# Ichoran/dbce-video-cpp

Measured on AMD Instinct MI355X. Metric: frames/s + raw-pixel GB/s, 4096x3072 U8 encode+decode round-trip, higher is better.
Workload: dtype u8

## Files before the change

### dbde-video-cpp_amd/csrc/dbde_kernels.hip

```cpp
#include "dbde_kernels.h"

#include "dbde_bits.h"
#include "dbde_device.h"


namespace dbde {

#ifndef DBDE_DIAG_LATE
#define DBDE_DIAG_LATE 34
#endif
#ifdef DBDE_DIAG
#define SF_DECL uint64_t sfd[10] = {0, 0, 0, 0, 0, 0, 0, 0, 0, 0}
#define SF_MARK(i) do { if (threadIdx.x == 0) sfd[i] = wall_clock64(); } while (0)
#define SF_DRAIN() asm volatile("s_waitcnt vmcnt(0) lgkmcnt(0)" ::: "memory")
#define SF_FLUSH(diag, last)                                                                          \
    do {                                                                                              \
        if (threadIdx.x == 0 && (diag)) {                                                             \
            atomicMax(&(diag)[0], ~(unsigned long long)sfd[0]);                                       \
            for (int i_ = 1; i_ < 10; i_++) atomicAdd(&(diag)[i_], (unsigned long long)sfd[i_]);      \
            atomicAdd(&(diag)[10], 1ull);                                                             \
            atomicMax(&(diag)[11], (unsigned long long)sfd[last]);                                    \
            atomicMax(&(diag)[12], (unsigned long long)sfd[0]);                                       \
            atomicAdd(&(diag)[13], (unsigned long long)sfd[0]);                                       \
        }                                                                                             \
// ... 1869 lines not shown
        uint32_t dsum = 0, dbad = 0;
        if (2u * (uint32_t)tid < n_tiles) { const uint32_t d = darr[te]; dsum += d; dbad |= d > 8u ? 1u : 0u; }
        if (2u * (uint32_t)tid + 1u < n_tiles) { const uint32_t d = darr[te + 1u]; dsum += d; dbad |= d > 8u ? 1u : 0u; }
        dsum = wave_sum(dsum);
        const bool wbad = __any((int)dbad);
        if (lane == 0) { s_idx[wave][0] = dsum; s_idx[wave][1] = wbad ? 1u : 0u; }
        __syncthreads();
        SF_MARK(1);
        unsigned long long *rec = p.fuse_rec + (size_t)f * cpf;
        const unsigned long long tag = (unsigned long long)p.fuse_epoch << 32;
        if (tid == 0 && !((p.fuse_flags & 1u) && (cf & 1u))) {
            uint32_t mine = 0, mbad = 0;
#pragma unroll
            for (int k = 0; k < G::kWaves; k++) { mine += s_idx[k][0]; mbad |= s_idx[k][1]; }
            __hip_atomic_store(&rec[cf], tag | ((unsigned long long)mbad << 31) | mine, __ATOMIC_RELAXED, __HIP_MEMORY_SCOPE_AGENT);
        }
        {
            const uint64_t t_start = wall_clock64();
            uint32_t before = 0, total = 0, flag = 0;
            auto take = [&](const uint32_t base, unsigned long long w) __attribute__((always_inline)) {
                const uint32_t k = base + (uint32_t)lane;
                bool got = k >= cpf || (w >> 32) == (tag >> 32);
                for (;;) {
                    if (__all((int)got)) break;
                    if (wall_clock64() - t_start > 3000ull) {
                        uint64_t miss = __ballot((int)!got);
                        while (miss) {
                            const uint32_t kk = (uint32_t)__builtin_ctzll(miss);
                            miss &= miss - 1ull;
                            const uint32_t c_lo = dec_chunk_begin(p.geom, base + kk), c_hi = dec_chunk_begin(p.geom, base + kk + 1u);
                            uint32_t sm = 0, bd = 0;
#pragma unroll
                            for (uint32_t j = 0; j < 8u; j += 4u) {
                                const uint32_t q = c_lo + (uint32_t)lane * 8u + j;
                                if (q < c_hi) {
                                    uint32_t x;
                                    __builtin_memcpy(&x, darr + q, 4);
                                    const uint32_t keep = c_hi - q;
                                    if (keep < 4u) x &= 0xFFFFFFFFu >> (8u * (4u - keep));
                                    bd |= depth_bytes_bad(x, 1u);
                                    sm += __builtin_amdgcn_sad_u8(x, 0u, 0u);
                                }
                            }
                            sm = wave_sum(sm);
                            const bool anyb = __any((int)(bd != 0u));
                            if ((uint32_t)lane == kk) { w = tag | ((unsigned long long)(anyb ? 1u : 0u) << 31) | sm; got = true; }
                        }
                        break;
                    }
                    __builtin_amdgcn_s_sleep(1);
                    if (!got) { w = __hip_atomic_load(&rec[k], __ATOMIC_RELAXED, __HIP_MEMORY_SCOPE_AGENT); got = (w >> 32) == (tag >> 32); }
                }
                const uint32_t v = k < cpf ? (uint32_t)w & 0x7FFFFFFFu : 0u;
                total += v;
                before += k < cf ? v : 0u;
                flag |= k < cpf ? (uint32_t)(w >> 31) & 1u : 0u;
            };
            constexpr uint32_t kStride = 64u * (uint32_t)G::kWaves;
            for (uint32_t base = 64u * (uint32_t)wave; base < cpf; base += 2u * kStride) {
                const uint32_t kA = base + (uint32_t)lane, kB = kA + kStride;
                const unsigned long long wA = kA < cpf ? __hip_atomic_load(&rec[kA], __ATOMIC_RELAXED, __HIP_MEMORY_SCOPE_AGENT) : 0ull;
                const unsigned long long wB = kB < cpf ? __hip_atomic_load(&rec[kB], __ATOMIC_RELAXED, __HIP_MEMORY_SCOPE_AGENT) : 0ull;
                take(base, wA);
                if (base + kStride < cpf) take(base + kStride, wB);
            }
            before = wave_sum(before); total = wave_sum(total);
            const bool anyflag = __any((int)flag);
            if (lane == 0) { s_idx[wave][2] = before; s_idx[wave][3] = total | (anyflag ? 0x80000000u : 0u); }
        }
        SF_MARK(2);
        __syncthreads();
        uint32_t before = 0, total = 0, flag = 0;
#pragma unroll
        for (int k = 0; k < G::kWaves; k++) { before += s_idx[k][2]; total += s_idx[k][3] & 0x7FFFFFFFu; flag |= s_idx[k][3] >> 31; }
        uint32_t mine = 0;
#pragma unroll
        for (int k = 0; k < G::kWaves; k++) mine += s_idx[k][0];
        const bool okf = nb == (int32_t)T && nm == (int32_t)T && n64 == (int32_t)total && !flag &&
                         in_extent(foff, need + 8ull * total, p.stream_bytes);
        if (record) {
            res->u64s = (field == 2u && okf) ? 2u : 0xFFFFFFFFu;
            res->pad_ = 0; res->index = index; res->elapsed_ns = elapsed;
            res->consumed = okf ? need + 8ull * total : 20ull;
        }
        if (!okf) return;
        w_begin = before;
        w_end = before + mine;
        __syncthreads();
        SF_MARK(3);
    } else {
        const uint32_t ok = p.frame_ok[f];
        const uint32_t *co = p.chunk_off + (size_t)f * (p.chunks_per_frame + 1u) + cf;
        w_begin = co[0]; w_end = co[1];
        asm volatile("" :: "s"(ok), "s"(w_begin), "s"(w_end), "s"((uint32_t)foff));
        if (!ok) return;
    }

    const uint32_t t0 = t_begin + 2u * (uint32_t)tid;
    const bool hasA = 2u * (uint32_t)tid < n_tiles, hasB = 2u * (uint32_t)tid + 1u < n_tiles;
    const uint8_t *depth_arr = fb + 24;
    const uint8_t *min_arr = fb + 28 + p.T;

    const uint32_t chunk_words = w_end - w_begin;
    const uint8_t *src = fb + 32ull + 2ull * p.T + 8ull * w_begin;
    const uint32_t shift = (uint32_t)(reinterpret_cast<uintptr_t>(src) & 15u);
    const uint8_t *asrc = src - shift;
    const uint32_t n16 = (shift + 8u * chunk_words + 15u) >> 4;
    const bool swz = chunk_words == 8u * n_tiles || chunk_words == 4u * n_tiles || chunk_words == 7u * n_tiles;
    const uint32_t n16r = (n16 + 15u) & ~15u;
    const uint8_t *s_end = p.stream + p.stream_bytes;
    const uint32_t n16_dma = (asrc + 16ull * n16 <= s_end) ? n16 : n16 - 1u;
#pragma unroll
    for (int j = 0; j < G::kPieces; j++) {
        const uint32_t i = (uint32_t)tid + (uint32_t)j * G::kThreads;
        const uint32_t src_slot = swz ? swz16(i) : i;
        if (i < n16r && src_slot < n16_dma) {
            const uint32_t wave_slot0 = (uint32_t)j * G::kThreads + (uint32_t)wave * 64u;
            __builtin_amdgcn_global_load_lds(
                (const __attribute__((address_space(1))) void *)(asrc + 16ull * src_slot),
                (__attribute__((address_space(3))) void *)(&s_in[2u * wave_slot0]), 16, 0, 2 );
        }
    }
    if (n16_dma != n16 && tid < 16) {
        const uint8_t *b = asrc + 16ull * n16_dma + (uint32_t)tid;
        reinterpret_cast<uint8_t *>(s_in)[16u * (swz ? swz16(n16_dma) : n16_dma) + (uint32_t)tid] = b < s_end ? *b : (uint8_t)0;
    }
    SF_MARK(4);
    uint32_t dA = 0, dB = 0, mA = 0, mB = 0;
    if (hasB && ((reinterpret_cast<uintptr_t>(depth_arr + t0) | reinterpret_cast<uintptr_t>(min_arr + t0)) & 1u) == 0u) {
        const uint32_t d2 = *reinterpret_cast<const uint16_t *>(depth_arr + t0);
        const uint32_t m2 = *reinterpret_cast<const uint16_t *>(min_arr + t0);
        dA = d2 & 0xFFu; dB = d2 >> 8; mA = m2 & 0xFFu; mB = m2 >> 8;
    } else {
        if (hasA) { dA = depth_arr[t0]; mA = min_arr[t0]; }
        if (hasB) { dB = depth_arr[t0 + 1]; mB = min_arr[t0 + 1]; }
    }

    asm volatile("s_waitcnt vmcnt(0) lgkmcnt(0)" ::: "memory");
    SF_MARK(5);
    uint32_t chunk_total;
    const uint32_t incl = block_scan_incl<G::kWaves>(dA + dB, s_wave_tot, lane, wave, chunk_total);
    SF_MARK(6);
    const uint32_t offA = incl - (dA + dB), offB = offA + dA;

    uint32_t va[16], vb[16];
    const uint8_t *s_img = reinterpret_cast<const uint8_t *>(s_in);
    const uint32_t bA = shift + 8u * offA, bB = shift + 8u * offB;
    const bool all8 = swz && (shift & 7u) == 0u && __all((int)((dA == 8u || !hasA) && (dB == 8u || !hasB)));
    const bool flat = __all((int)((dA | dB) == 0u));
    if (flat) {
#pragma unroll
        for (int i = 0; i < 16; i++) { va[i] = mA * 0x01010101u; vb[i] = mB * 0x01010101u; }
    } else if (all8) {
        unpack_tile_d8_from_lds(s_img, bA, mA, va);
        unpack_tile_d8_from_lds(s_img, bB, mB, vb);
    } else {
        if (swz) {
            unpack_tile_from_lds<true>(s_img, bA, dA, mA, va);
            unpack_tile_from_lds<true>(s_img, bB, dB, mB, vb);
        } else {
            unpack_tile_from_lds<false>(s_img, bA, dA, mA, va);
            unpack_tile_from_lds<false>(s_img, bB, dB, mB, vb);
        }
    }

    SF_MARK(7);
    uint8_t *img = p.images + (size_t)f * p.frame_pixels;
    if (IMG == kImgDirect) {
        if (hasA) {
            const uint32_t ty = t0 / p.w, tx = t0 - ty * p.w;
            uint8_t *base = img + (size_t)(8u * tx);
#pragma unroll
            for (int r = 0; r < 8; r++) {
                const int yy = 8 * (int)ty + r;
                if (yy < p.H) {
                    u32x4_t o;
                    o[0] = va[2 * r]; o[1] = va[2 * r + 1]; o[2] = vb[2 * r]; o[3] = vb[2 * r + 1];
                    __builtin_nontemporal_store(o, reinterpret_cast<u32x4_t *>(base + (size_t)yy * (size_t)p.W));
                }
            }
        }
        SF_MARK(8);
        SF_DRAIN();
        SF_MARK(9);
        if (INDEX == kIdxFused) SF_FLUSH(p.diag, 9);
        return;
    }

    if (IMG == kImgTiles) {
        if (hasA) store_tile_generic(img, p.W, p.H, p.w, t0, va);
        if (hasB) store_tile_generic(img, p.W, p.H, p.w, t0 + 1u, vb);
        return;
    }

    const bool whole_rows = p.geom.pieces == 1u;
    const uint32_t ty0 = whole_rows ? t_begin / p.w : cf / p.geom.pieces;
    const uint32_t tx0 = whole_rows ? 0u : (cf - ty0 * p.geom.pieces) * kChunkTiles;
    const uint32_t wspan = whole_rows ? p.w : n_tiles;
    const uint32_t Wu = (uint32_t)p.W, y0 = 8u * ty0;
    const uint32_t tile_rows = whole_rows ? n_tiles / p.w : 1u;
    const uint32_t y_end = y0 + 8u * tile_rows < (uint32_t)p.H ? y0 + 8u * tile_rows : (uint32_t)p.H;
    const uint32_t x_valid = Wu - 8u * tx0 < 8u * wspan ? Wu - 8u * tx0 : 8u * wspan;
    uint8_t *g_first = img + (size_t)y0 * (size_t)p.W + (size_t)(8u * tx0);
    const uint32_t g7 = (uint32_t)(reinterpret_cast<uintptr_t>(g_first) & 127u);
    uint8_t *s_px = reinterpret_cast<uint8_t *>(s_in);
    const bool a8 = ((g7 | Wu) & 7u) == 0u;
    if (!a8 && !whole_rows) {
        if (hasA) store_tile_generic(img, p.W, p.H, p.w, t0, va);
        if (hasB) store_tile_generic(img, p.W, p.H, p.w, t0 + 1u, vb);
        return;
    }
    if (whole_rows && ((uint32_t)(reinterpret_cast<uintptr_t>(img) & 15u) | (Wu & 15u)) == 0u && chunk_words != 8u * n_tiles) {
        if (hasA) {
            const uint32_t iD = 2u * (uint32_t)tid, rowD = iD / wspan, colD = iD - rowD * wspan;
            uint8_t *base = img + (size_t)(8u * colD);
#pragma unroll
            for (int r = 0; r < 8; r++) {
                const uint32_t yy = y0 + 8u * rowD + (uint32_t)r;
                if (yy < (uint32_t)p.H) {
                    u32x4_t o;
                    o[0] = va[2 * r]; o[1] = va[2 * r + 1]; o[2] = vb[2 * r]; o[3] = vb[2 * r + 1];
                    __builtin_nontemporal_store(o, reinterpret_cast<u32x4_t *>(base + (size_t)yy * (size_t)p.W));
                }
            }
        }
        return;
    }
    __syncthreads();
    const uint32_t iA = 2u * (uint32_t)tid;
    const uint32_t rowA = iA / wspan, colA = iA - rowA * wspan;
    const uint32_t rowB = colA + 1u == wspan ? rowA + 1u : rowA, colB = colA + 1u == wspan ? 0u : colA + 1u;
    const uint32_t nA = 8u * colA + 8u <= x_valid ? 8u : x_valid - 8u * colA;
    const uint32_t nB = 8u * colB + 8u <= x_valid ? 8u : x_valid - 8u * colB;
    const bool all_rows = y0 + 8u * tile_rows <= (uint32_t)p.H;
    const bool plain = all_rows && __all((int)((!hasA || nA == 8u) && (!hasB || nB == 8u)));
    if (a8) {
        const uint32_t l_pitch = 8u * kChunkTiles + 128u;
        const uint32_t aA = whole_rows ? g7 + 8u * rowA * Wu + 8u * colA : 8u * colA;
        const uint32_t aB = whole_rows ? g7 + 8u * rowB * Wu + 8u * colB : 8u * colB;
        auto row_term = [&](uint32_t r) -> uint32_t {
            return whole_rows ? r * Wu : ((g7 + r * Wu) & 127u) + r * l_pitch;
        };
        if (plain) {
            if (hasA) {
#pragma unroll
                for (int r = 0; r < 8; r++) lds_store_u64_any(s_px, aA + row_term((uint32_t)r), va[2 * r], va[2 * r + 1]);
            }
            if (hasB) {
#pragma unroll
                for (int r = 0; r < 8; r++) lds_store_u64_any(s_px, aB + row_term((uint32_t)r), vb[2 * r], vb[2 * r + 1]);
            }
        } else {
#pragma unroll
            for (int r = 0; r < 8; r++) {
                const uint32_t rt = row_term((uint32_t)r);
                if (hasA && y0 + 8u * rowA + (uint32_t)r < y_end) {
                    if (nA == 8u) lds_store_u64_any(s_px, aA + rt, va[2 * r], va[2 * r + 1]);
                    else lds_store_bytes(s_px, aA + rt, ((uint64_t)va[2 * r + 1] << 32) | va[2 * r], nA);
                }
                if (hasB && y0 + 8u * rowB + (uint32_t)r < y_end) {
                    if (nB == 8u) lds_store_u64_any(s_px, aB + rt, vb[2 * r], vb[2 * r + 1]);
                    else lds_store_bytes(s_px, aB + rt, ((uint64_t)vb[2 * r + 1] << 32) | vb[2 * r], nB);
                }
            }
        }
        asm volatile("s_waitcnt lgkmcnt(0)" ::: "memory");
        __syncthreads();
        const uint32_t n_ranges = whole_rows ? 1u : y_end - y0;
        for (uint32_t s = 0; s < n_ranges; s++) {
            uint8_t *g0 = g_first + (size_t)s * Wu;
            const uint32_t bytes = whole_rows ? (y_end - y0) * Wu : x_valid;
            const uint32_t head = (uint32_t)(reinterpret_cast<uintptr_t>(g0) & 127u);
            uint8_t *a0 = g0 - head;
            const uint8_t *l0 = s_px + (whole_rows ? 0u : s * l_pitch);
            const uint32_t n_blocks = (head + bytes + 15u) >> 4;
            for (uint32_t j = (uint32_t)tid; j < n_blocks; j += (uint32_t)G::kThreads) {
                if (16u * j + 16u <= head || 16u * j >= head + bytes) continue;
                if (16u * j >= head && 16u * j + 16u <= head + bytes) {
                    const u32x4_t q = *reinterpret_cast<const u32x4_t *>(l0 + 16u * j);
                    __builtin_nontemporal_store(q, reinterpret_cast<u32x4_t *>(a0 + 16ull * j));
                } else {
#pragma unroll
                    for (uint32_t b = 0; b < 16u; b++) {
                        const uint32_t o = 16u * j + b;
                        if (o >= head && o < head + bytes) a0[o] = l0[o];
                    }
                }
            }
        }
        return;
    }
    const uint32_t P = 8u * wspan + 16u;
    const uint32_t aA = 8u * rowA * P + 8u * colA, aB = 8u * rowB * P + 8u * colB;
    if (hasA) {
#pragma unroll
        for (int r = 0; r < 8; r++) lds_store_u64_any(s_px, aA + (uint32_t)r * P, va[2 * r], va[2 * r + 1]);
    }
    if (hasB) {
#pragma unroll
        for (int r = 0; r < 8; r++) lds_store_u64_any(s_px, aB + (uint32_t)r * P, vb[2 * r], vb[2 * r + 1]);
    }
    asm volatile("s_waitcnt lgkmcnt(0)" ::: "memory");
    __syncthreads();
    if (hasA && colA <= 1u) {
#pragma unroll
        for (int r = 0; r < 8; r++) {
            const uint32_t ry = 8u * rowA + (uint32_t)r;
            if (ry != 0u) lds_store_u64_any(s_px, (ry - 1u) * P + Wu + 8u * colA, va[2 * r], va[2 * r + 1]);
        }
    }
    if (hasB && colB <= 1u) {
#pragma unroll
        for (int r = 0; r < 8; r++) {
            const uint32_t ry = 8u * rowB + (uint32_t)r;
            if (ry != 0u) lds_store_u64_any(s_px, (ry - 1u) * P + Wu + 8u * colB, vb[2 * r], vb[2 * r + 1]);
        }
    }
    asm volatile("s_waitcnt lgkmcnt(0)" ::: "memory");
    __syncthreads();
    {
        const uint32_t bytes = (y_end - y0) * Wu;
        uint8_t *a0 = g_first - g7;
        const uint32_t n_blocks = (g7 + bytes + 15u) >> 4;
        const uint32_t lds0 = (uint32_t)(uintptr_t)(__attribute__((address_space(3))) const uint8_t *)s_px;
        const uint32_t last_n = (g7 + bytes) & 15u;
        for (uint32_t j0 = (uint32_t)tid; j0 < n_blocks; j0 += 4u * (uint32_t)G::kThreads) {
            uint64_t d01[4], d23[4];
            uint32_t d4[4], a[4];
            bool live[4];
#pragma unroll
            for (uint32_t k = 0; k < 4u; k++) {
                const uint32_t j = j0 + k * (uint32_t)G::kThreads;
                live[k] = j < n_blocks && 16u * j + 16u > g7;
                const uint32_t o = live[k] && 16u * j > g7 ? 16u * j - g7 : 0u;
                uint32_t col;
                const uint32_t row = div_magic(o, Wu, p.magic_W, col);
                a[k] = lds0 + row * P + col;
                const uint32_t a4 = a[k] & ~3u;
                asm volatile("ds_read2_b32 %0, %3 offset1:1\n\tds_read2_b32 %1, %3 offset0:2 offset1:3\n\tds_read_b32 %2, %3 offset:16"
                             : "=&v"(d01[k]), "=&v"(d23[k]), "=&v"(d4[k]) : "v"(a4) : "memory");
            }
            asm volatile("s_waitcnt lgkmcnt(0)" : "+v"(d01[0]), "+v"(d23[0]), "+v"(d4[0]), "+v"(d01[1]), "+v"(d23[1]), "+v"(d4[1]),
                         "+v"(d01[2]), "+v"(d23[2]), "+v"(d4[2]), "+v"(d01[3]), "+v"(d23[3]), "+v"(d4[3]) :: "memory");
#pragma unroll
            for (uint32_t k = 0; k < 4u; k++) {
                const uint32_t j = j0 + k * (uint32_t)G::kThreads;
                const uint32_t w0 = (uint32_t)d01[k], w1 = (uint32_t)(d01[k] >> 32), w2 = (uint32_t)d23[k], w3 = (uint32_t)(d23[k] >> 32);
                u32x4_t q;
                q[0] = __builtin_amdgcn_alignbyte(w1, w0, a[k]);
                q[1] = __builtin_amdgcn_alignbyte(w2, w1, a[k]);
                q[2] = __builtin_amdgcn_alignbyte(w3, w2, a[k]);
                q[3] = __builtin_amdgcn_alignbyte(d4[k], w3, a[k]);
                if (!live[k]) continue;
                const bool first = 16u * j < g7, last = 16u * j + 16u > g7 + bytes;
                if (!first && !last) {
                    __builtin_nontemporal_store(q, reinterpret_cast<u32x4_t *>(a0 + 16ull * j));
                } else {
                    uint8_t *dst = first ? g_first : a0 + 16ull * j;
                    uint32_t n = first ? 16u - (g7 & 15u) : last_n;
                    if (first && last) n = bytes;
                    uint64_t lo = ((uint64_t)q[1] << 32) | q[0], hi = ((uint64_t)q[3] << 32) | q[2];
                    if (n & 8u) { store_u64_any(dst, lo); dst += 8; lo = hi; }
                    if (n & 4u) { const uint32_t v = (uint32_t)lo; __builtin_memcpy(dst, &v, 4); dst += 4; lo >>= 32; }
                    if (n & 2u) { const uint16_t v = (uint16_t)lo; __builtin_memcpy(dst, &v, 2); dst += 2; lo >>= 16; }
                    if (n & 1u) *dst = (uint8_t)lo;
                }
            }
        }
    }
}

struct MidMeta {
    uint32_t d, mn;
    uint32_t nb, nm, n64;
};

#ifndef DBDE_MID_WAVES
#define DBDE_MID_WAVES 6
#endif
template <int THREADS, bool STAGED>
__global__ __launch_bounds__(THREADS, THREADS == 1024 ? 4 : DBDE_MID_WAVES) void decode_mid_kernel(DecParams p) {
    constexpr int NW = THREADS / 64;
    __shared__ uint32_t s_tot[2][NW];
    __shared__ uint32_t s_incl[2][THREADS];
    constexpr uint32_t kMidSlot = 80u;
    __shared__ __attribute__((aligned(16))) uint8_t s_lds[THREADS * kMidSlot];
    __shared__ uint32_t s_ok[THREADS];
    __shared__ uint32_t s_bad[2];
    const uint32_t tid = threadIdx.x, lane = tid & 63u, wave = tid >> 6;
    const uint32_t T = p.T, fpw = (uint32_t)THREADS / T;
    const uint32_t fl = tid / T, t = tid - fl * T;
    const uint32_t n_frames = p.n_chunks;
    const uint32_t n_groups = (n_frames + fpw - 1u) / fpw, G = gridDim.x;
    const bool slot = fl < fpw;
    const uint32_t first = slot ? fl * T : 0u;
    const uint64_t need = 32ull + 2ull * T;
    const uint8_t *s_end = p.stream + p.stream_bytes;
    const uint32_t ty = t / p.w, tx = t - ty * p.w;
    const uint32_t Wu = (uint32_t)p.W, x0 = 8u * tx;
    const uint32_t rm = Wu - x0 < 8u ? Wu - x0 : 8u;
    const uint32_t rv = (uint32_t)p.H - 8u * ty < 8u ? (uint32_t)p.H - 8u * ty : 8u;
    const uint32_t tile_off = 8u * ty * Wu + x0;
    const bool want_results = p.results != nullptr;

    auto is_active = [&](uint32_t g) -> bool { return slot && g < n_groups && g * fpw + fl < n_frames; };
    auto get_foff = [&](uint32_t g) -> uint64_t { return is_active(g) ? p.frame_offsets[g * fpw + fl] : 0ull; };
    auto get_meta = [&](uint32_t g, uint64_t foff) -> MidMeta {
        MidMeta m;
        m.d = 0; m.mn = 0; m.nb = 0; m.nm = 0; m.n64 = 0;
        const bool active = is_active(g);
        const uint8_t *fb = p.stream + foff;
        if (active && in_extent(foff, need, p.stream_bytes)) {
            m.d = fb[24u + t]; m.mn = fb[28u + T + t];
            __builtin_memcpy(&m.nb, fb + 20, 4); __builtin_memcpy(&m.nm, fb + 24 + T, 4); __builtin_memcpy(&m.n64, fb + 28 + 2ull * T, 4);
        }
        return m;
    };

    if (STAGED && tid == 0u) { s_bad[0] = 0u; s_bad[1] = 0u; }
    uint32_t g = blockIdx.x;
    uint64_t foff_cur = get_foff(g), foff_nxt = get_foff(g + G);
    auto settle = [&](const MidMeta &x, uint32_t &dm, uint32_t &n64x) {
        dm = x.d | (x.mn << 8);
        n64x = ((int32_t)x.nb == (int32_t)T && (int32_t)x.nm == (int32_t)T) ? x.n64 : 0xFFFFFFFFu;
    };
    uint32_t dm, n64x;
    settle(get_meta(g, foff_cur), dm, n64x);
    for (uint32_t par = 0; g < n_groups; g += G, par ^= 1u) {
        MidMeta m_nxt = get_meta(g + G, foff_nxt);
        uint64_t foff_nn = get_foff(g + 2u * G);
        const bool active = is_active(g);
        const uint32_t f = g * fpw + fl;
        const uint64_t foff = foff_cur;
        const bool in_range = active && in_extent(foff, need, p.stream_bytes);
        const uint32_t d = dm & 0xFFu, mn = dm >> 8;
        const uint32_t item = in_range ? (d | (d > 8u ? 1u << 20 : 0u)) : 0u;
        const uint32_t w_incl = wave_scan_incl(item);
        s_incl[par][tid] = w_incl;
        if (lane == 63u) s_tot[par][wave] = w_incl;
        lds_barrier();
        if (STAGED && tid == 0u) s_bad[par ^ 1u] = 0u;
        auto pref = [&](uint32_t x) -> uint32_t {
            uint32_t a = s_incl[par][x];
#pragma unroll
            for (int k = 0; k < NW - 1; k++) a += (uint32_t)k < (x >> 6) ? s_tot[par][k] : 0u;
            return a;
        };
        const uint32_t base = first ? pref(active ? first - 1u : 0u) : 0u;
        const uint32_t upto = pref(active ? first + T - 1u : 0u);
        const uint32_t mine = pref(tid);
        const uint32_t total = (upto - base) & 0xFFFFFu, n_bad = (upto - base) >> 20;
        const uint32_t prefix = (mine - item - base) & 0xFFFFFu;
        const bool ok = in_range && n64x == total && n_bad == 0u && in_extent(foff, need + 8ull * total, p.stream_bytes);
        uint32_t h_field = 0;
        uint64_t h_index = 0, h_elapsed = 0;
        const bool record = active && t == 0u && want_results;
        if (record && in_extent(foff, 20, p.stream_bytes)) {
            const uint8_t *fb = p.stream + foff;
            __builtin_memcpy(&h_field, fb, 4); __builtin_memcpy(&h_index, fb + 4, 8); __builtin_memcpy(&h_elapsed, fb + 12, 8);
        }
        const uint8_t *pay = p.stream + foff + need + 8ull * prefix;
        const uint32_t poff = (uint32_t)(reinterpret_cast<uintptr_t>(pay) & 3u);
        const uint8_t *psrc = pay - poff;
        const uint32_t npc_all = (8u * d + poff + 15u) >> 4;
        const bool whole = ok && d != 0u && psrc + 16u * npc_all <= s_end;
        const uint32_t npc = whole ? npc_all : 0u;
        u32x4_t q0 = {0u, 0u, 0u, 0u}, q1 = q0, q2 = q0, q3 = q0, q4 = q0;
        if (npc > 0u) __builtin_memcpy(&q0, psrc, 16);
        if (npc > 1u) __builtin_memcpy(&q1, psrc + 16, 16);
        if (npc > 2u) __builtin_memcpy(&q2, psrc + 32, 16);
        if (npc > 3u) __builtin_memcpy(&q3, psrc + 48, 16);
        if (npc > 4u) __builtin_memcpy(&q4, psrc + 64, 16);
        asm volatile("" : "+v"(q0), "+v"(q1), "+v"(q2), "+v"(q3), "+v"(q4),
                          "+v"(m_nxt.d), "+v"(m_nxt.mn), "+v"(m_nxt.nb), "+v"(m_nxt.nm), "+v"(m_nxt.n64), "+v"(foff_nn),
                          "+v"(h_field), "+v"(h_index), "+v"(h_elapsed) :: "memory");
        const uint32_t slot = kMidSlot * tid;
        {
            u32x4_t *sl = reinterpret_cast<u32x4_t *>(s_lds + slot);
            if (npc > 0u) sl[0] = q0;
            if (npc > 1u) sl[1] = q1;
            if (npc > 2u) sl[2] = q2;
            if (npc > 3u) sl[3] = q3;
            if (npc > 4u) sl[4] = q4;
        }
        if (ok && d != 0u && !whole) {
            for (uint32_t b = 0; b < 8u * d; b++) s_lds[slot + poff + b] = pay[b];
        }
        uint32_t v[16];
#pragma unroll
        for (int i = 0; i < 16; i++) v[i] = 0;
        if (ok) unpack_tile_from_lds<false>(s_lds, slot + poff, d, mn, v);
        if (STAGED) lds_barrier();
        if (ok) {
            uint8_t *dst = p.images + (size_t)f * p.frame_pixels + tile_off;
            const uint32_t px0 = ((uint32_t)(reinterpret_cast<uintptr_t>(p.images) + (size_t)(g * fpw) * p.frame_pixels) & 15u) +
                                 fl * (uint32_t)p.frame_pixels + tile_off;
#pragma unroll
            for (int r = 0; r < 8; r++) {
                const uint32_t lo = v[2 * r], hi = v[2 * r + 1];
                if (STAGED) {
                    if ((uint32_t)r < rv) {
                        const uint32_t a = px0 + (uint32_t)r * Wu;
                        if ((Wu & 7u) == 0u) lds_store_u64_any(s_lds, a, lo, hi);
                        else {
                            *reinterpret_cast<uint32_t *>(s_lds + a) = lo;
                            if (rm == 8u) *reinterpret_cast<uint32_t *>(s_lds + a + 4u) = hi;
                        }
                    }
                } else if ((uint32_t)r < rv) {
                    uint8_t *row = dst + (size_t)r * Wu;
                    const uint64_t q = ((uint64_t)hi << 32) | lo;
                    if (rm == 8u) store_u64_any(row, q);
                    else {
#pragma unroll
                        for (uint32_t k = 0; k < 8u; k++)
                            if (k < rm) row[k] = (uint8_t)(q >> (8u * k));
                    }
                }
            }
        }
        if (STAGED) {
            if (active && t == 0u) { s_ok[fl] = ok ? 1u : 0u; if (!ok) s_bad[par] = 1u; }
            lds_barrier();
            const uint32_t P = (uint32_t)p.frame_pixels;
            const uint32_t nfr = n_frames - g * fpw < fpw ? n_frames - g * fpw : fpw;
            uint8_t *g0 = p.images + (size_t)(g * fpw) * p.frame_pixels;
            const uint32_t sh = (uint32_t)(reinterpret_cast<uintptr_t>(g0) & 15u);
            const uint32_t nbytes = nfr * P;
            if (s_bad[par] == 0u) {
                const uint32_t n_blocks = (sh + nbytes + 15u) >> 4;
                for (uint32_t j = tid; j < n_blocks; j += (uint32_t)THREADS) {
                    uint8_t *dst = g0 - sh + 16ull * j;
                    if (16u * j >= sh && 16u * j + 16u <= sh + nbytes) {
                        const u32x4_t q = *reinterpret_cast<const u32x4_t *>(s_lds + 16u * j);
                        __builtin_nontemporal_store(q, reinterpret_cast<u32x4_t *>(dst));
                    } else {
#pragma unroll
                        for (uint32_t k = 0; k < 4u; k++) {
                            const uint32_t o = 16u * j + 4u * k;
                            if (o >= sh && o < sh + nbytes) *reinterpret_cast<uint32_t *>(dst + 4u * k) = *reinterpret_cast<const uint32_t *>(s_lds + o);
                        }
                    }
                }
            } else {
                for (uint32_t u = tid; 4u * u < nbytes; u += (uint32_t)THREADS) {
                    const uint32_t o = 4u * u;
                    if (s_ok[o / P]) *reinterpret_cast<uint32_t *>(g0 + o) = *reinterpret_cast<const uint32_t *>(s_lds + sh + o);
                }
            }
        }
        if (record) {
            FrameResultDev *r = reinterpret_cast<FrameResultDev *>(p.results) + f;
            r->u64s = (h_field == 2u && ok) ? 2u : 0xFFFFFFFFu;
            r->pad_ = 0;
            r->index = h_index;
            r->elapsed_ns = f64_to_u64_x86(__longlong_as_double((long long)h_elapsed));
            r->consumed = ok ? need + 8ull * total : 20ull;
        }
        foff_cur = foff_nxt; foff_nxt = foff_nn;
        settle(m_nxt, dm, n64x);
    }
}

void decode_mid_blocks_per_cu(int (&per_cu)[2][3]) {
    auto ask = [](auto kernel, int threads) {
        int n = 0;
        if (hipOccupancyMaxActiveBlocksPerMultiprocessor(&n, kernel, threads, 0) != hipSuccess || n < 1) n = 1;
        return n;
    };
    per_cu[0][0] = ask(decode_mid_kernel<256, false>, 256);
    per_cu[0][1] = ask(decode_mid_kernel<512, false>, 512);
    per_cu[0][2] = ask(decode_mid_kernel<1024, false>, 1024);
    per_cu[1][0] = ask(decode_mid_kernel<256, true>, 256);
    per_cu[1][1] = ask(decode_mid_kernel<512, true>, 512);
    per_cu[1][2] = ask(decode_mid_kernel<1024, true>, 1024);
}

hipError_t launch_decode_mid(const DecParams &p, uint32_t n_frames, uint32_t n_cu, const int (&per_cu)[2][3], hipStream_t s) {
    DecParams q = p;
    q.n_chunks = n_frames;
    const uint32_t th = mid_decode_threads_for(p.T), per_wg = th / p.T;
    uint32_t groups = (n_frames + per_wg - 1u) / per_wg;
    const bool staged = p.W % 4 == 0 && (reinterpret_cast<uintptr_t>(p.images) & 3u) == 0u;
    auto go = [&](auto kernel, uint32_t threads) {
        const int wg = per_cu[staged ? 1 : 0][threads == 256u ? 0 : (threads == 512u ? 1 : 2)];
        const uint32_t resident = n_cu ? n_cu * (uint32_t)wg : 3u;
        hipLaunchKernelGGL(kernel, dim3(groups < resident ? groups : resident), dim3(threads), 0, s, q);
    };
    if (staged) {
        if (th == 256u) go(decode_mid_kernel<256, true>, 256u);
        else if (th == 512u) go(decode_mid_kernel<512, true>, 512u);
        else go(decode_mid_kernel<1024, true>, 1024u);
    } else {
        if (th == 256u) go(decode_mid_kernel<256, false>, 256u);
        else if (th == 512u) go(decode_mid_kernel<512, false>, 512u);
        else go(decode_mid_kernel<1024, false>, 1024u);
    }
    return hipGetLastError();
}

__device__ __forceinline__ u32x4_t frame_block(const uint8_t *m, uint32_t pay0, const uint8_t *pay, uint32_t meta, uint32_t o) {
    u32x4_t q;
    if (o + 16u <= meta) {
        q = *reinterpret_cast<const u32x4_t *>(m + o);
    } else if ((meta & 15u) == 0u) {
        q = *reinterpret_cast<const u32x4_t *>(pay + (o - meta));
    } else {
        const int po = (int)o - (int)meta;
        const uint32_t a = (uint32_t)((int)pay0 + po), a4 = a & ~3u;
        uint64_t d01, d23;
        uint32_t d4;
        asm volatile("ds_read2_b32 %0, %3 offset1:1\n\tds_read2_b32 %1, %3 offset0:2 offset1:3\n\tds_read_b32 %2, %3 offset:16\n\ts_waitcnt lgkmcnt(0)"
                     : "=&v"(d01), "=&v"(d23), "=&v"(d4) : "v"(po < 0 ? pay0 & ~3u : a4) : "memory");
        const uint32_t w0 = (uint32_t)d01, w1 = (uint32_t)(d01 >> 32), w2 = (uint32_t)d23, w3 = (uint32_t)(d23 >> 32);
        q[0] = __builtin_amdgcn_alignbyte(w1, w0, a);
        q[1] = __builtin_amdgcn_alignbyte(w2, w1, a);
        q[2] = __builtin_amdgcn_alignbyte(w3, w2, a);
        q[3] = __builtin_amdgcn_alignbyte(d4, w3, a);
        if (po < 0) {
#pragma unroll
            for (uint32_t i = 0; i < 4u; i++) {
                uint32_t x = 0;
#pragma unroll
                for (uint32_t j = 0; j < 4u; j++) {
                    const uint32_t at = o + 4u * i + j;
                    x |= (uint32_t)(at < meta ? m[at] : pay[at - meta]) << (8u * j);
                }
                q[i] = x;
            }
        }
    }
    return q;
}

template <int THREADS>
struct FramesLds {
    static constexpr uint32_t kCap = 2u * THREADS;
    static constexpr uint32_t kMaxFrames = kCap / 65u;
    static constexpr uint32_t kMetaBytes = 2u * kCap + 48u * (kMaxFrames + 1u);
};

template <int THREADS>
__global__ __launch_bounds__(THREADS) void encode_frames_kernel(EncParams p) {
    typedef FramesLds<THREADS> G;
    constexpr int NW = THREADS / 64;
    __shared__ __attribute__((aligned(16))) uint64_t s_px[G::kCap * 8u + THREADS];
    __shared__ __attribute__((aligned(16))) uint8_t s_meta[G::kMetaBytes];
    __shared__ uint32_t s_tot[NW];
    __shared__ uint32_t s_fbase[G::kMaxFrames + 1], s_fend[G::kMaxFrames + 1];
    const uint32_t tid = threadIdx.x, lane = tid & 63u, wave = tid >> 6;
    const uint32_t T = p.T, F = G::kCap / T;
    const uint32_t f0 = blockIdx.x * F;
    const uint32_t nf = p.n_chunks - f0 < F ? p.n_chunks - f0 : F;
    const uint32_t P = (uint32_t)p.frame_pixels, W = (uint32_t)p.W;
    const uint32_t meta = 32u + 2u * T, mpitch = (meta + 15u) & ~15u;

    {
        const uint8_t *src = p.images + (size_t)f0 * P;
        const uint32_t n16 = nf * (P >> 4);
        for (uint32_t i = tid; i < n16; i += THREADS)
            __builtin_amdgcn_global_load_lds((const __attribute__((address_space(1))) void *)(src + 16ull * i),
                                             (__attribute__((address_space(3))) void *)(s_px + 2u * (i - lane)), 16, 0, 2 );
        asm volatile("s_waitcnt vmcnt(0)" ::: "memory");
    }
    __syncthreads();

    const uint8_t *s_img = reinterpret_cast<const uint8_t *>(s_px);
    uint32_t v[2][16], mn[2], d[2], fl[2], tt[2];
    bool has[2];
#pragma unroll
// ... 503 lines not shown
```

Baseline: 120,100.

## Rework decode LDS-to-global writeout with incremental addressing and row-tail copy

Replaces the per-block row-tail duplication (done by threads owning column 0/1 blocks) with a per-row copy that places the start of each next row after the previous row's end in LDS. Block addressing now uses an incremental stride in place of a magic division per block, and LDS reads use three 64-bit reads. Partial first and last blocks are split out of the main loop and handled by two dedicated threads. The goal is less integer arithmetic and branching in the store loop; the cost is an extra LDS pass for row tails and more complex edge handling.

New measurement: 120,100, median of 5. Within noise of the previous version (+0.0%).

```diff
diff --git a/dbde-video-cpp_amd/csrc/dbde_kernels.hip b/dbde-video-cpp_amd/csrc/dbde_kernels.hip
--- a/dbde-video-cpp_amd/csrc/dbde_kernels.hip
+++ b/dbde-video-cpp_amd/csrc/dbde_kernels.hip
@@ -2195,70 +2195,89 @@
     }
     asm volatile("s_waitcnt lgkmcnt(0)" ::: "memory");
     __syncthreads();
-    if (hasA && colA <= 1u) {
-#pragma unroll
-        for (int r = 0; r < 8; r++) {
-            const uint32_t ry = 8u * rowA + (uint32_t)r;
-            if (ry != 0u) lds_store_u64_any(s_px, (ry - 1u) * P + Wu + 8u * colA, va[2 * r], va[2 * r + 1]);
-        }
-    }
-    if (hasB && colB <= 1u) {
-#pragma unroll
-        for (int r = 0; r < 8; r++) {
-            const uint32_t ry = 8u * rowB + (uint32_t)r;
-            if (ry != 0u) lds_store_u64_any(s_px, (ry - 1u) * P + Wu + 8u * colB, vb[2 * r], vb[2 * r + 1]);
-        }
-    }
-    asm volatile("s_waitcnt lgkmcnt(0)" ::: "memory");
+    const uint32_t lds0 = (uint32_t)(uintptr_t)(__attribute__((address_space(3))) const uint8_t *)s_px;
+    const uint32_t n_rows = y_end - y0;
+    for (uint32_t ry = (uint32_t)tid + 1u; ry < n_rows; ry += (uint32_t)G::kThreads) {
+        const uint32_t *head = reinterpret_cast<const uint32_t *>(s_px + ry * P);
+        uint32_t *tail = reinterpret_cast<uint32_t *>(s_px + (ry - 1u) * P + (Wu & ~3u));
+        const uint32_t s4 = Wu & 3u, sh = 4u - s4;
+        const uint32_t h0 = head[0], h1 = head[1], h2 = head[2], h3 = head[3];
+        if (s4 == 0u) {
+            tail[0] = h0; tail[1] = h1; tail[2] = h2; tail[3] = h3;
+        } else {
+            const uint32_t t = tail[0] << (8u * sh);
+            tail[0] = __builtin_amdgcn_alignbyte(h0, t, sh);
+            tail[1] = __builtin_amdgcn_alignbyte(h1, h0, sh);
+            tail[2] = __builtin_amdgcn_alignbyte(h2, h1, sh);
+            tail[3] = __builtin_amdgcn_alignbyte(h3, h2, sh);
+            tail[4] = h3 >> (8u * sh);
+        }
+    }
     __syncthreads();
     {
-        const uint32_t bytes = (y_end - y0) * Wu;
+        const uint32_t bytes = n_rows * Wu;
         uint8_t *a0 = g_first - g7;
-        const uint32_t n_blocks = (g7 + bytes + 15u) >> 4;
-        const uint32_t lds0 = (uint32_t)(uintptr_t)(__attribute__((address_space(3))) const uint8_t *)s_px;
-        const uint32_t last_n = (g7 + bytes) & 15u;
-        for (uint32_t j0 = (uint32_t)tid; j0 < n_blocks; j0 += 4u * (uint32_t)G::kThreads) {
-            uint64_t d01[4], d23[4];
-            uint32_t d4[4], a[4];
-            bool live[4];
+        const uint32_t j_lo = (g7 + 15u) >> 4, j_hi = (g7 + bytes) >> 4;
+        constexpr uint32_t kStep = 16u * (uint32_t)G::kThreads;
+        uint32_t r_step;
+        const uint32_t q_step = div_magic(kStep, Wu, p.magic_W, r_step);
+        const uint32_t l_step = q_step * P + r_step, l_wrap = P - Wu;
+        auto read_block = [&](uint32_t a, uint64_t &x01, uint64_t &x23, uint64_t &x45) {
+            asm volatile("ds_read_b64 %0, %3\n\tds_read_b64 %1, %3 offset:8\n\tds_read_b64 %2, %3 offset:16"
+                         : "=&v"(x01), "=&v"(x23), "=&v"(x45) : "v"(a & ~7u) : "memory");
+        };
+        auto block_of = [&](uint32_t a, uint64_t x01, uint64_t x23, uint64_t x45) -> u32x4_t {
+            const bool hi = (a & 4u) != 0u;
+            const uint32_t e0 = hi ? (uint32_t)(x01 >> 32) : (uint32_t)x01, e1 = hi ? (uint32_t)x23 : (uint32_t)(x01 >> 32);
+            const uint32_t e2 = hi ? (uint32_t)(x23 >> 32) : (uint32_t)x23, e3 = hi ? (uint32_t)x45 : (uint32_t)(x23 >> 32);
+            const uint32_t e4 = hi ? (uint32_t)(x45 >> 32) : (uint32_t)x45;
+            u32x4_t q;
+            q[0] = __builtin_amdgcn_alignbyte(e1, e0, a);
+            q[1] = __builtin_amdgcn_alignbyte(e2, e1, a);
+            q[2] = __builtin_amdgcn_alignbyte(e3, e2, a);
+            q[3] = __builtin_amdgcn_alignbyte(e4, e3, a);
+            return q;
+        };
+        uint32_t j = j_lo + (uint32_t)tid, col;
+        uint32_t la = lds0 + div_magic(16u * j - g7, Wu, p.magic_W, col) * P + col;
+        for (; j < j_hi; j += 4u * (uint32_t)G::kThreads) {
+            uint64_t x01[4], x23[4], x45[4];
+            uint32_t a[4];
 #pragma unroll
             for (uint32_t k = 0; k < 4u; k++) {
-                const uint32_t j = j0 + k * (uint32_t)G::kThreads;
-                live[k] = j < n_blocks && 16u * j + 16u > g7;
-                const uint32_t o = live[k] && 16u * j > g7 ? 16u * j - g7 : 0u;
-                uint32_t col;
-                const uint32_t row = div_magic(o, Wu, p.magic_W, col);
-                a[k] = lds0 + row * P + col;
-                const uint32_t a4 = a[k] & ~3u;
-                asm volatile("ds_read2_b32 %0, %3 offset1:1\n\tds_read2_b32 %1, %3 offset0:2 offset1:3\n\tds_read_b32 %2, %3 offset:16"
-                             : "=&v"(d01[k]), "=&v"(d23[k]), "=&v"(d4[k]) : "v"(a4) : "memory");
-            }
-            asm volatile("s_waitcnt lgkmcnt(0)" : "+v"(d01[0]), "+v"(d23[0]), "+v"(d4[0]), "+v"(d01[1]), "+v"(d23[1]), "+v"(d4[1]),
-                         "+v"(d01[2]), "+v"(d23[2]), "+v"(d4[2]), "+v"(d01[3]), "+v"(d23[3]), "+v"(d4[3]) :: "memory");
+                a[k] = j + k * (uint32_t)G::kThreads < j_hi ? la : lds0;
+                read_block(a[k], x01[k], x23[k], x45[k]);
+                col += r_step;
+                la += l_step;
+                if (col >= Wu) { col -= Wu; la += l_wrap; }
+            }
+            asm volatile("s_waitcnt lgkmcnt(0)" : "+v"(x01[0]), "+v"(x23[0]), "+v"(x45[0]), "+v"(x01[1]), "+v"(x23[1]), "+v"(x45[1]),
+                         "+v"(x01[2]), "+v"(x23[2]), "+v"(x45[2]), "+v"(x01[3]), "+v"(x23[3]), "+v"(x45[3]) :: "memory");
 #pragma unroll
             for (uint32_t k = 0; k < 4u; k++) {
-                const uint32_t j = j0 + k * (uint32_t)G::kThreads;
-                const uint32_t w0 = (uint32_t)d01[k], w1 = (uint32_t)(d01[k] >> 32), w2 = (uint32_t)d23[k], w3 = (uint32_t)(d23[k] >> 32);
-                u32x4_t q;
-                q[0] = __builtin_amdgcn_alignbyte(w1, w0, a[k]);
-                q[1] = __builtin_amdgcn_alignbyte(w2, w1, a[k]);
-                q[2] = __builtin_amdgcn_alignbyte(w3, w2, a[k]);
-                q[3] = __builtin_amdgcn_alignbyte(d4[k], w3, a[k]);
-                if (!live[k]) continue;
-                const bool first = 16u * j < g7, last = 16u * j + 16u > g7 + bytes;
-                if (!first && !last) {
-                    __builtin_nontemporal_store(q, reinterpret_cast<u32x4_t *>(a0 + 16ull * j));
-                } else {
-                    uint8_t *dst = first ? g_first : a0 + 16ull * j;
-                    uint32_t n = first ? 16u - (g7 & 15u) : last_n;
-                    if (first && last) n = bytes;
-                    uint64_t lo = ((uint64_t)q[1] << 32) | q[0], hi = ((uint64_t)q[3] << 32) | q[2];
-                    if (n & 8u) { store_u64_any(dst, lo); dst += 8; lo = hi; }
-                    if (n & 4u) { const uint32_t v = (uint32_t)lo; __builtin_memcpy(dst, &v, 4); dst += 4; lo >>= 32; }
-                    if (n & 2u) { const uint16_t v = (uint16_t)lo; __builtin_memcpy(dst, &v, 2); dst += 2; lo >>= 16; }
-                    if (n & 1u) *dst = (uint8_t)lo;
-                }
-            }
+                const uint32_t jk = j + k * (uint32_t)G::kThreads;
+                if (jk < j_hi)
+                    __builtin_nontemporal_store(block_of(a[k], x01[k], x23[k], x45[k]), reinterpret_cast<u32x4_t *>(a0 + 16u * jk));
+            }
+        }
+        const bool first = (uint32_t)tid == 0u && (g7 & 15u) != 0u;
+        const bool last = (uint32_t)tid == (uint32_t)G::kThreads - 1u && ((g7 + bytes) & 15u) != 0u && 16u * j_hi >= g7;
+        if (first || last) {
+            const uint32_t o = first ? 0u : 16u * j_hi - g7;
+            uint32_t c0;
+            uint64_t x01, x23, x45;
+            const uint32_t a = lds0 + div_magic(o, Wu, p.magic_W, c0) * P + c0;
+            read_block(a, x01, x23, x45);
+            asm volatile("s_waitcnt lgkmcnt(0)" : "+v"(x01), "+v"(x23), "+v"(x45) :: "memory");
+            const u32x4_t q = block_of(a, x01, x23, x45);
+            uint8_t *dst = g_first + o;
+            uint32_t n = first ? 16u - (g7 & 15u) : (g7 + bytes) & 15u;
+            if (n > bytes - o) n = bytes - o;
+            uint64_t lo = ((uint64_t)q[1] << 32) | q[0], hi = ((uint64_t)q[3] << 32) | q[2];
+            if (n & 8u) { store_u64_any(dst, lo); dst += 8; lo = hi; }
+            if (n & 4u) { const uint32_t v = (uint32_t)lo; __builtin_memcpy(dst, &v, 4); dst += 4; lo >>= 32; }
+            if (n & 2u) { const uint16_t v = (uint16_t)lo; __builtin_memcpy(dst, &v, 2); dst += 2; lo >>= 16; }
+            if (n & 1u) *dst = (uint8_t)lo;
         }
     }
 }
```
